# mafintosh/dat-replication-protocol

Hardware: AMD Instinct MI355X
Metric: decoded Change frames/sec + wire GB/s (whole node) at 1/2/4/8 MI355X (higher is better)
Workload: dtype u8

## Files before the change

### dat-replication-protocol_amd/csrc/drp_decode_spec.hip

```cpp
#include "drp_spec.h"

#include <algorithm>
#include <cstdio>
#include <cstdlib>
#include <vector>

namespace drp {
namespace spec {

#ifndef DRP_K1_WAVES
#define DRP_K1_WAVES 8
#endif
#ifndef DRP_EMIT_WAVES
#define DRP_EMIT_WAVES 5
#endif
#ifndef DRP_KSTRONG
#define DRP_KSTRONG 4
#endif
constexpr int KSTRONG = DRP_KSTRONG;
struct Img {
  const uint8_t *lds;
  const uint8_t *g;
  uint64_t A, se;
  bool local = true;
// ... 579 lines not shown
    const uint64_t L1 = H1 ? ((1ull << (63 - __builtin_clzll(H1))) - 1) : 0ull;
    const uint64_t L0 = H1 ? ~0ull : (H0 ? ((1ull << (63 - __builtin_clzll(H0))) - 1) : 0ull);
    S0 = H0 & ~(F0 & L0);
    S1 = H1 & ~(F1 & L1);
    if (far && any_above(H0, H1, tid)) {
      g = NONE;
      R = NONE;
      n = 0;
    }
  }
  uint64_t E = g;
  bool rs = false;
  PHASE(1);
  link<false>(m, s1, g, NONE, E, R, n, xr, xf, P.overflow, &rs);
  uint32_t need = (E == NONE && defer && !any_above(S0, S1, tid)) ? 1u : 0u;
  uint32_t js = (is_pos(E) && E < s1) ? tid + 1 : 0u;
  block_max2_u32(need, js, xf2);
  bool moved = false;
  for (uint32_t it = 0; need && it < 3; it++) {
    moved = true;
    if (E == NONE && defer && !any_above(S0, S1, tid)) {
      while (defer) {
        const uint32_t o = (uint32_t)__builtin_ctzll(defer);
        defer &= defer - 1;
        uint64_t r;
        uint32_t k;
        bool f;
        if (strong<false>(m, lb + o, s1, r, k, f, P.kstrong_hbm) == S_OK) {
          g = lb + o;
          E = g;
          R = r;
          n = k;
          break;
        }
      }
    }
    link<false>(m, s1, g, NONE, E, R, n, xr, xf, P.overflow, &rs);
    need = (E == NONE && defer && !any_above(S0, S1, tid)) ? 1u : 0u;
    js = (is_pos(E) && E < s1) ? tid + 1 : 0u;
    block_max2_u32(need, js, xf2);
  }
  PHASE(2);
  {
    bool after;
    if (!moved) {
      after = any_from(S0, S1, js);
    } else {
      after = block_max_u32(g != NONE && tid + 1 > js ? 1u : 0u, xf2) != 0;
    }
    if (js && after) {
      const uint64_t Ea = E, Ra = R;
      const uint32_t na = n;
      const bool rsa = rs;
      const bool mine = tid + 1 > js;
      E = NONE;
      R = NONE;
      n = 0;
      link<false>(m, s1, mine ? g : NONE, NONE, E, R, n, xr, xf, P.overflow, &rs);
      const uint32_t nb = block_sum_u32(mine ? (n & 0xFFFFu) : 0u, xf2);
      if (nb < 2 || !mine) {
        E = Ea;
        R = Ra;
        n = na;
        rs = rsa;
      }
    }
  }
  PHASE(3);
  {
    const bool carrier = is_pos(E) && E >= lb && E < s1 && E < G.se;
    const uint64_t ix = t * NT + tid;
    P.ent[ix] = carrier ? (uint8_t)((E - lb) | (rs ? 0x40u : 0u)) : (uint8_t)0xFF;
    P.ent_n[ix] = carrier ? (uint8_t)(n & 0xFFFFu) : (uint8_t)0;
    P.ent_c[ix] = carrier ? (uint8_t)(n >> 16) : (uint8_t)0;
  }
  if (tid == NT - 1) P.claim[t] = (R == NONE || ((R & MARK_TERM) && (R & M_ERR))) ? C_ID : R;
  }
}

#ifndef DRP_FCAP
#define DRP_FCAP 512
#endif
constexpr uint32_t FCAP = DRP_FCAP;
constexpr uint16_t NX_TAILB = 0xFFFB, NX_TAILC = 0xFFFC;
constexpr uint32_t RX_NONE = 0xFFFFFFFFu;
constexpr uint32_t RX_DEAD = 0xFFFFFFFEu;
constexpr uint32_t RX_FAR = 0x80000000u;
constexpr uint32_t RX_TERM = 0x40000000u;
static_assert(IMG < 0x4000, "node offsets are 14-bit");
__device__ __forceinline__ bool rx_node(uint32_t x) { return x < RX_TERM; }
__device__ __forceinline__ uint32_t rx_off(uint32_t x) { return x >> 16; }

__device__ __forceinline__ uint32_t le2_bytes(uint32_t x) { return ~(((x | 0x80808080u) - 0x03030303u) | x) & 0x80808080u; }
__device__ __forceinline__ uint32_t gather_msb(uint32_t a, uint32_t b, uint32_t c, uint32_t d) {
  const uint32_t lo = __builtin_amdgcn_udot4(a, 0x08040201u, __builtin_amdgcn_udot4(b, 0x80402010u, 0u, false), false);
  const uint32_t hi = __builtin_amdgcn_udot4(c, 0x08040201u, __builtin_amdgcn_udot4(d, 0x80402010u, 0u, false), false);
  return (lo >> 7) | (hi << 1);
}
__device__ __forceinline__ uint32_t masks16(const uint4 v) {
  constexpr uint32_t H = 0x80808080u;
  const uint32_t m = gather_msb(v.x & H, v.y & H, v.z & H, v.w & H);
  const uint32_t s = gather_msb(le2_bytes(v.x), le2_bytes(v.y), le2_bytes(v.z), le2_bytes(v.w));
  return m | (s << 16);
}


__device__ __forceinline__ bool change_fills(const uint32_t *w32, uint32_t po, uint32_t pl, uint32_t lim,
                                             uint32_t off = 0, uint32_t found = 0) {
#pragma unroll 1
  for (uint32_t f = 0; f < 8u && off < pl; f++) {
    const uint32_t q = po + off;
    if (q + 12u > lim) return false;
    const uint32_t d = q >> 2, sh = (q & 3u) * 8u;
    const uint32_t a0 = w32[d], a1 = w32[d + 1], a2 = w32[d + 2];
    const uint32_t w = __builtin_amdgcn_alignbit(a1, a0, sh), wn = __builtin_amdgcn_alignbit(a2, a1, sh);
    const uint32_t b0 = w & 0xFFu, tag = b0 >> 3;
    const bool num = tag - 3u <= 2u;
    if (b0 >= 0x80u || tag - 1u > 5u || (b0 & 7u) != (num ? 0u : 2u)) return false;
    const uint32_t x = __builtin_amdgcn_alignbit(wn, w, 8);
    const uint32_t tm = ~x & 0x80808080u;
    uint32_t k2;
    uint64_t v = (x & 0x7Fu) | ((x >> 1) & 0x3F80u) | ((x >> 2) & 0x1FC000u) | ((x >> 3) & 0xFE00000u);
    if (tm) {
      k2 = ((uint32_t)__builtin_ctz(tm) >> 3) + 1u;
      v &= (1u << (7u * k2)) - 1u;
    } else {
      const uint32_t b5 = (wn >> 8) & 0xFFu;
      if (b5 & 0x80u) return false;
      k2 = 5u;
      v |= (uint64_t)b5 << 28;
    }
    if (k2 + 1u > pl - off) return false;
    if (num) {
      found |= 1u << (tag - 2u);
      off += 1u + k2;
    } else {
      const uint32_t o2 = off + 1u + k2;
      if (v > (uint64_t)(pl - o2)) return false;
      if (tag == 2u) found |= 1u;
      off = o2 + (uint32_t)v;
    }
  }
  return off == pl && found == 15u;
}

__device__ __forceinline__ uint32_t change_fills_win(const uint32_t *w32, uint32_t po, uint32_t pl, uint32_t lim,
                                                     uint32_t off, uint32_t found) {
  const uint32_t q = po + off;
  if (q + 36u > lim) return 2u;
  const uint32_t d = q >> 2, sh = (q & 3u) * 8u;
  uint32_t a[9];
#pragma unroll
  for (int i = 0; i < 9; i++) a[i] = w32[d + i];
  uint64_t x[4];
#pragma unroll
  for (int i = 0; i < 4; i++)
    x[i] = (uint64_t)__builtin_amdgcn_alignbit(a[2 * i + 1], a[2 * i], sh) |
           ((uint64_t)__builtin_amdgcn_alignbit(a[2 * i + 2], a[2 * i + 1], sh) << 32);
  uint32_t used = 0;
#pragma unroll
  for (int f = 0; f < 4; f++) {
    const uint32_t b0 = (uint32_t)x[0] & 0xFFu, tag = b0 >> 3;
    const uint64_t y = x[0] >> 8;
    const uint64_t tm = ~y & 0x8080808080ull;
    if (b0 >= 0x80u || !tm) return 0u;
    const uint32_t k2 = ((uint32_t)__builtin_ctzll(tm) >> 3) + 1u;
    const uint64_t v = ((y & 0x7Full) | ((y >> 1) & 0x3F80ull) | ((y >> 2) & 0x1FC000ull) | ((y >> 3) & 0xFE00000ull) |
                        ((y >> 4) & 0x7F0000000ull)) & ((1ull << (7u * k2)) - 1ull);
    if (tag - 3u <= 2u && (b0 & 7u) == 0u) {
      found |= 1u << (tag - 2u);
      const uint32_t s = 1u + k2;
      used += s;
      if (off + used > pl) return 0u;
      const uint32_t b = 8u * s;
      x[0] = (x[0] >> b) | (x[1] << (64u - b));
      x[1] = (x[1] >> b) | (x[2] << (64u - b));
      x[2] = (x[2] >> b) | (x[3] << (64u - b));
      x[3] >>= b;
      continue;
    }
    if (b0 == 0x32u) {
      return (found == 15u && (uint64_t)off + used + 1u + k2 + v == (uint64_t)pl) ? 1u : 0u;
    }
    if (b0 == 0x0Au || b0 == 0x12u) return 2u;
    return 0u;
  }
  return 2u;
}

__device__ __forceinline__ uint32_t fwalk(const uint32_t *lnd, uint32_t x, uint32_t s1r, uint32_t &n) {
  n = 0;
  uint32_t i = x & 0xFFFFu;
#pragma unroll 1
  for (;;) {
    const uint32_t nd = lnd[i], id = nd >> 30, c = nd & 0xFFFFu, q = (nd >> 16) & 0x3FFFu;
    if (id == 3) return RX_DEAD;
    if (c == NX_TAILC) return RX_TERM | i;
    n += 1u + ((id == 1) << 16) - (id == 0);
    if (c == NX_TAILB) return RX_TERM | i;
    if (c == NX_FAR || c == NX_NEAR) return RX_FAR | i;
    if (q >= s1r) return c == NX_DEAD ? RX_DEAD : (c | (q << 16));
    if (c == NX_DEAD) return RX_DEAD;
    i = c;
  }
}

__device__ __forceinline__ bool flink(const uint32_t *lnd, uint32_t s1r, uint32_t g, uint32_t &E, uint32_t &R,
                                      uint32_t &n, bool &rs, uint32_t *wl, uint32_t *fl, uint32_t *overflow,
                                      unsigned long long *stats = nullptr, uint32_t cap = ~0u) {
  const uint32_t tid = threadIdx.x, lane = tid & 63u, wid = tid >> 6;
  const uint64_t below = (1ull << lane) - 1ull;
#pragma unroll 1
  for (uint32_t round = 0;; round++) {
    const bool carrier = rx_node(E) && rx_off(E) < s1r;
    const uint64_t cm = __ballot(carrier);
    const uint64_t bm = cm & below;
    const uint32_t j = bm ? 63u - (uint32_t)__builtin_clzll(bm) : 0u;
    const uint32_t xj = (uint32_t)__builtin_amdgcn_ds_bpermute((int)(j << 2), (int)R);
    if constexpr (NT == 2 * WAVE) {
      if (lane == 0) wl[wid] = cm ? (uint32_t)__builtin_amdgcn_readlane((int)R, 63 - __builtin_clzll(cm)) : RX_NONE;
      bsync();
    }
    const uint32_t prev = (NT == 2 * WAVE && wid == 1) ? wl[0] : RX_NONE;
    const uint32_t ex = bm ? xj : prev;
    const bool r = ex >= RX_DEAD;
    const uint32_t En = r ? g : ex;
    const bool ch = En != E;
    const bool relevant = ch && (carrier || (rx_node(En) && rx_off(En) < s1r));
    const uint64_t any = __ballot(relevant);
    bool more = any != 0;
    if constexpr (NT == 2 * WAVE) {
      if (lane == 0) fl[wid] = any != 0;
      bsync();
      more = (fl[0] | fl[1]) != 0;
    }
    rs = r;
    if (more && round + 1 >= cap) return true;
    if (!more) {
      if (stats && tid == 0) {
        atomicAdd(&stats[56], (unsigned long long)(round + 1));
        atomicMax(&stats[57], (unsigned long long)(round + 1));
        if (round + 1 > 8) atomicAdd(&stats[58], 1ull);
      }
      if (ch) {
        E = En;
        R = En;
        n = 0;
      }
      break;
    }
    if (round > NT + 2) {
      if (tid == 0) atomicOr(overflow, F_WAIT);
      break;
    }
    if (ch) {
      E = En;
      if (rx_node(E) && rx_off(E) < s1r) R = fwalk(lnd, E, s1r, n);
      else {
        R = E;
        n = 0;
      }
    }
  }
  return false;
}



constexpr uint32_t HV = HALO / SEGB;
struct FastLds {
  union {
    struct {
      uint64_t lmw[NT + HV];
      uint64_t dmw[NT];
      uint16_t loff[NT + HV];
      uint32_t hmx[HALO / 16 + 1];
      uint16_t lpos[FCAP];
      uint32_t lnd[FCAP > NT + 1 ? FCAP : NT + 1];
      uint8_t lal[FCAP];
      uint32_t lsucc[FCAP];
    };
    __attribute__((aligned(16))) uint8_t img[IMG + 32];
  };
  uint32_t fls[NT];
  uint32_t xw[8];
  uint32_t xf[2 * NT / WAVE], wl[NT / WAVE], fl[NT / WAVE];
  uint64_t xm[4];
#ifdef DRP_K1_PAD
  uint8_t pad[DRP_K1_PAD];
#endif
};
static_assert(sizeof(FastLds) <= SPEC_BUF, "spec_claims runs the edge form in its image buffer");


#ifndef DRP_FL_CAP
#define DRP_FL_CAP 6
#endif
constexpr uint32_t JT_C_ID = 2u << 30, JT_TERM = 1u << 30, JT_NONE = 0xFFFFu;
template <uint32_t NTT>
__device__ __forceinline__ uint32_t fast_claims_jump(const DecodeParams &P, uint64_t t, uint64_t A, FastLds &S, uint32_t g,
                                                  uint32_t ttotal, uint32_t total, uint32_t &eb_o, uint32_t &en_o,
                                                  uint32_t &ecn_o, uint64_t &cl_o) {
  const uint32_t tid = threadIdx.x, lane = tid & 63u, wid = tid >> 6;
  constexpr uint32_t KPT = FCAP / NTT;
  uint16_t *nx = reinterpret_cast<uint16_t *>(S.lmw);
  uint32_t *gl = reinterpret_cast<uint32_t *>(S.dmw);
  uint32_t *lnd = S.lnd;
  if (P.stats && tid == 0) atomicAdd(&P.stats[60], 1ull);
  const uint64_t gm = __ballot(g != RX_NONE);
  if (lane == 0) S.xm[wid] = gm;
  gl[tid] = g;
  bsync();
  const uint64_t G0 = S.xm[0], G1 = NTT == 2 * WAVE ? S.xm[1] : 0ull;
  uint32_t yn[KPT], yt[KPT];
#pragma unroll
  for (uint32_t j = 0; j < KPT; j++) {
    const uint32_t i = tid + j * NTT;
    yn[j] = JT_NONE;
    yt[j] = JT_C_ID;
    if (i < ttotal) {
      const uint32_t o = S.lpos[i], th = o / SEGB;
      uint32_t cnt;
      const uint32_t x = fwalk(lnd, i, (th + 1u) * SEGB, cnt);
      if (rx_node(x)) {
        const uint32_t k = x & 0xFFFFu;
        if (S.lpos[k] >= TILE) yt[j] = S.lpos[k];
        else yn[j] = k;
      } else if (x == RX_DEAD) {
        const uint64_t a0 = th + 1u < 64u ? G0 & (~0ull << (th + 1u)) : 0ull;
        const uint64_t a1 = th + 1u < 64u ? G1 : (th + 1u < 128u ? G1 & (~0ull << (th + 1u - 64u)) : 0ull);
        const uint32_t k = a0 ? (uint32_t)__builtin_ctzll(a0) : (a1 ? 64u + (uint32_t)__builtin_ctzll(a1) : NTT);
        if (k < NTT) yn[j] = gl[k] & 0xFFFFu;
      } else if (x & RX_FAR) {
        yt[j] = S.lsucc[x & 0xFFFFu];
      } else if (x & RX_TERM) {
        yt[j] = JT_TERM | S.lpos[x & 0xFFFFu];
      }
    } else if (i < total) {
      yt[j] = S.lpos[i];
    }
  }
  bsync();
#pragma unroll
  for (uint32_t j = 0; j < KPT; j++) {
    const uint32_t i = tid + j * NTT;
    if (i < total) {
      nx[i] = (uint16_t)yn[j];
      lnd[i] = yt[j];
    }
  }
  bsync();
#pragma unroll 1
  for (uint32_t round = 0; round < 10u; round++) {
    uint32_t chm = 0;
#pragma unroll
    for (uint32_t j = 0; j < KPT; j++) {
      const uint32_t i = tid + j * NTT;
      if (i < total && nx[i] != JT_NONE) {
        const uint32_t a = nx[i], b = nx[a];
        yn[j] = b;
        yt[j] = b == JT_NONE ? lnd[a] : 0u;
        chm |= 1u << j;
      }
    }
    const uint64_t any = __ballot(chm != 0);
    if (lane == 0) S.fl[wid] = any != 0;
    bsync();
    uint32_t more = 0;
#pragma unroll
    for (uint32_t w = 0; w < NTT / WAVE; w++) more |= S.fl[w];
#pragma unroll
    for (uint32_t j = 0; j < KPT; j++)
      if ((chm >> j) & 1u) {
        const uint32_t i = tid + j * NTT;
        nx[i] = (uint16_t)yn[j];
        if (yn[j] == JT_NONE) lnd[i] = yt[j];
      }
    bsync();
    if (!more) break;
  }
  const uint64_t ix = t * NTT + tid;
  eb_o = 0xFFu;
  en_o = 0;
  ecn_o = 0;
  P.ent[ix] = 0xFF;
  P.ent_n[ix] = 0;
  P.ent_c[ix] = 0;
  cl_o = 0;
  if (tid == NTT - 1) {
    uint64_t cl = C_ID;
    if (G0 | G1) {
      const uint32_t k = G0 ? (uint32_t)__builtin_ctzll(G0) : 64u + (uint32_t)__builtin_ctzll(G1);
      const uint32_t s0 = gl[k] & 0xFFFFu;
      const uint32_t code = nx[s0] == JT_NONE ? lnd[s0] : JT_C_ID;
      if (code == JT_C_ID) cl = C_ID;
      else if (code & JT_TERM) cl = MARK_TERM | (A + (code & ~JT_TERM));
      else cl = A + code;
    }
    P.claim[t] = cl;
    cl_o = cl;
  }
  return FC_OK;
}

#ifndef DRP_CREC_STAGE
#define DRP_CREC_STAGE 2
#endif
constexpr uint32_t CR_CAP = NT, CR_WORDS = 6, CR_TILE_WORDS = CR_CAP * CR_WORDS;
static_assert(CR_CAP == NT, "one frame per thread in the record decode");

__device__ __forceinline__ bool crec_general(const uint32_t *w32, uint32_t qa, uint32_t ke, uint32_t pl,
                                             uint32_t &num0, uint32_t &num1, uint32_t &num2, uint32_t &vo, bool &hv) {
  const uint32_t d = qa >> 2, sh = (qa & 3u) * 8u;
  uint32_t a[8];
#pragma unroll
  for (int i = 0; i < 8; i++) a[i] = w32[d + i];
  uint64_t x[4];
#pragma unroll
  for (int i = 0; i < 3; i++)
    x[i] = (uint64_t)__builtin_amdgcn_alignbit(a[2 * i + 1], a[2 * i], sh) |
           ((uint64_t)__builtin_amdgcn_alignbit(a[2 * i + 2], a[2 * i + 1], sh) << 32);
  x[3] = __builtin_amdgcn_alignbit(a[7], a[6], sh);
  uint32_t used = 0, nums[3];
#pragma unroll
  for (int f = 0; f < 3; f++) {
    const uint32_t b0 = (uint32_t)x[0] & 0xFFu;
    const uint64_t y = x[0] >> 8;
    const uint64_t tm = ~y & 0x8080808080ull;
    if (b0 != 0x18u + 8u * (uint32_t)f || !tm) return false;
    const uint32_t k2 = ((uint32_t)__builtin_ctzll(tm) >> 3) + 1u;
    const uint64_t v = ((y & 0x7Full) | ((y >> 1) & 0x3F80ull) | ((y >> 2) & 0x1FC000ull) | ((y >> 3) & 0xFE00000ull) |
                        ((y >> 4) & 0x7F0000000ull)) & ((1ull << (7u * k2)) - 1ull);
    if (v >> 32) return false;
    nums[f] = (uint32_t)v;
    const uint32_t s = 1u + k2, b = 8u * s;
    used += s;
    x[0] = (x[0] >> b) | (x[1] << (64u - b));
    x[1] = (x[1] >> b) | (x[2] << (64u - b));
    x[2] = (x[2] >> b) | (x[3] << (64u - b));
    x[3] >>= b;
  }
  num0 = nums[0];
  num1 = nums[1];
  num2 = nums[2];
  if (ke + used > pl) return false;
  hv = ke + used != pl;
  vo = 0;
  if (!hv) return true;
  const uint32_t b0 = (uint32_t)x[0] & 0xFFu;
  const uint64_t y = x[0] >> 8;
  const uint64_t tm = ~y & 0x80808080ull;
  if (b0 != 0x32u || !tm) return false;
  const uint32_t k2 = ((uint32_t)__builtin_ctzll(tm) >> 3) + 1u;
  const uint64_t v = ((y & 0x7Full) | ((y >> 1) & 0x3F80ull) | ((y >> 2) & 0x1FC000ull) | ((y >> 3) & 0xFE00000ull)) &
                     ((1ull << (7u * k2)) - 1ull);
  vo = ke + used + 1u + k2;
  return vo <= pl && v == (uint64_t)(pl - vo) && vo < 0x10000u;
}

__device__ __forceinline__ bool crec_frame(const uint32_t *w32, uint32_t o, uint32_t se_rel, uint32_t id, bool tailb,
                                           uint32_t (&w)[CR_WORDS]) {
  const uint32_t d = o >> 2, sh = (o & 3u) * 8u;
  const uint32_t a0 = w32[d], a1 = w32[d + 1], a2 = w32[d + 2];
  const uint32_t h = __builtin_amdgcn_alignbit(a1, a0, sh), hn = __builtin_amdgcn_alignbit(a2, a1, sh);
  const uint32_t k = ((uint32_t)__builtin_ctz((~h & 0x808080u) | 0x80000000u) >> 3) + 1u;
  const uint32_t L = ((h & 0x7Fu) | ((h >> 1) & 0x3F80u) | ((h >> 2) & 0x1FC000u)) & ((1u << (7u * k)) - 1u);
  const uint32_t po = o + k + 1u, pl = L - 1u;
  w[0] = po | (id << 14) | ((tailb ? 1u : 0u) << 16);
  w[1] = pl;
  w[2] = w[3] = w[4] = w[5] = 0;
  if (id != 1u) return true;
  const uint64_t x = (((uint64_t)hn << 32) | h) >> (8u * (k + 1u));
  const uint32_t b1 = (uint32_t)(x >> 8) & 0xFFu, b2 = (uint32_t)(x >> 16) & 0xFFu;
  const uint32_t kb = b1 < 0x80u ? 1u : (b2 < 0x80u ? 2u : 0u);
  const uint32_t klen = kb == 1u ? b1 : (b1 & 0x7Fu) | (b2 << 7);
  const uint32_t ke = 1u + kb + klen;
  uint32_t n0 = 0, n1 = 0, n2 = 0, vo = 0;
  bool hv = false, ok = ((uint32_t)x & 0xFFu) == 0x12u && kb && ke + 6u <= pl;
  const uint32_t qa = po + ke;
  ok = ok && qa + 36u <= se_rel;
  if (ok) {
    const uint32_t e = qa >> 2, s2 = (qa & 3u) * 8u;
    const uint32_t c0 = w32[e], c1 = w32[e + 1], c2 = w32[e + 2], c3 = w32[e + 3];
    const uint64_t y = (uint64_t)__builtin_amdgcn_alignbit(c1, c0, s2) | ((uint64_t)__builtin_amdgcn_alignbit(c2, c1, s2) << 32);
    const uint32_t y8 = __builtin_amdgcn_alignbit(c3, c2, s2) & 0xFFu;
    const bool one = (y & 0xFFull) == 0x18u && ((y >> 16) & 0xFFull) == 0x20u && ((y >> 32) & 0xFFull) == 0x28u &&
                     (y & 0x0000800080008000ull) == 0;
    if (one) {
      n0 = (uint32_t)(y >> 8) & 0xFFu;
      n1 = (uint32_t)(y >> 24) & 0xFFu;
      n2 = (uint32_t)(y >> 40) & 0xFFu;
      if (ke + 6u != pl) {
        const uint32_t d0 = (uint32_t)(y >> 56), vh = d0 < 0x80u ? 2u : (y8 < 0x80u ? 3u : 0u);
        const uint32_t vl = vh == 2u ? d0 : (d0 & 0x7Fu) | (y8 << 7);
        vo = ke + 6u + vh;
        hv = true;
        ok = ((uint32_t)(y >> 48) & 0xFFu) == 0x32u && vh && vo <= pl && vl == pl - vo && vo < 0x10000u;
      }
    } else {
      ok = crec_general(w32, qa, ke, pl, n0, n1, n2, vo, hv);
    }
  }
  w[0] |= ((hv ? 1u : 0u) << 17) | (kb << 18);
  w[2] = klen | (vo << 16);
  w[3] = n0;
  w[4] = n1;
  w[5] = n2;
  return ok;
}

__device__ __forceinline__ void fast_records(const DecodeParams &P, uint64_t t, FastLds &S, uint32_t E, uint32_t nf,
                                             uint32_t s1r, uint32_t se_rel, const uint4 (&v)[SEGB / 16],
                                             const uint4 &hv) {
  const uint32_t tid = threadIdx.x, lane = tid & 63u, wid = tid >> 6;
  const uint32_t ip = wave_scan_dpp(nf);
  if (lane == 63) S.xw[4 + wid] = ip;
  bsync();
  const uint32_t tot = NT == 2 * WAVE ? S.xw[4] + S.xw[5] : S.xw[4];
  if (tot > CR_CAP) return;
  uint32_t bad = 0;
  if (nf) {
    uint32_t slot = ip - nf + (wid ? S.xw[4] : 0u), cnt = 0, i = E & 0xFFFFu;
#pragma unroll 1
    for (uint32_t g = 0; g < 64u; g++) {
      const uint32_t nd = S.lnd[i], id = nd >> 30, c = nd & 0xFFFFu, q = (nd >> 16) & 0x3FFFu;
      if (id == 3u || c == NX_TAILC) break;
      if (id != 0u) {
        if (cnt < nf) S.fls[slot + cnt] = (uint32_t)S.lpos[i] | (id << 14) | ((c == NX_TAILB ? 1u : 0u) << 16);
        cnt++;
      }
      if (c >= NX_TAILB || q >= s1r) break;
      i = c;
    }
    bad = cnt != nf;
  }
  bsync();
  if (DRP_CREC_STAGE == 0) return;
  uint4 *im = reinterpret_cast<uint4 *>(S.img);
#pragma unroll
  for (uint32_t k = 0; k < SEGB / 16; k++) im[tid * (SEGB / 16) + k] = v[k];
  if (tid < HALO / 16) im[TILE / 16 + tid] = hv;
  if (tid < 2) im[IMG / 16 + tid] = make_uint4(0, 0, 0, 0);
  bsync();
  if (tid < tot && !bad) {
    const uint32_t f = S.fls[tid];
    uint32_t w[CR_WORDS];
    bad = !crec_frame(reinterpret_cast<const uint32_t *>(S.img), f & 0x3FFFu, min(se_rel, IMG), (f >> 14) & 3u,
                      (f >> 16) & 1u, w);
    uint32_t *rr = P.rec + t * CR_TILE_WORDS + tid;
    if (DRP_CREC_STAGE == 1) {
      if ((w[0] ^ w[2] ^ w[3] ^ w[4] ^ w[5]) == 0x7FFFFFFFu && !bad) rr[0] = w[1];
      bad = true;
    }
    if (!bad) {
      rr[0] = w[0];
      rr[CR_CAP] = w[1];
      if ((w[0] >> 14 & 3u) == 1u) {
#pragma unroll
        for (uint32_t k = 2; k < CR_WORDS; k++) rr[k * CR_CAP] = w[k];
      }
    }
  }
  const uint64_t bm = __ballot(bad);
  if (lane == 0) S.xw[6 + wid] = bm != 0;
  bsync();
  if (tid == 0) P.tile_rec[t] = (NT == 2 * WAVE ? S.xw[6] | S.xw[7] : S.xw[6]) ? REC_NONE : 0u;
}

__device__ __forceinline__ uint64_t range_bits(uint32_t base, uint32_t lo, uint32_t hi) {
  const uint32_t a = lo > base ? min(lo - base, 64u) : 0u, z = hi > base ? min(hi - base, 64u) : 0u;
  const uint64_t za = z >= 64u ? ~0ull : ((1ull << z) - 1ull), aa = a >= 64u ? ~0ull : ((1ull << a) - 1ull);
  return za & ~aa;
}

template <bool CF, bool EDGE, bool REC>
__device__ __forceinline__ uint32_t fast_claims(const DecodeParams &P, const TileGeo &G, uint64_t t, FastLds &S,
                                                uint32_t &eb_o, uint32_t &en_o, uint32_t &ecn_o, uint64_t &cl_o) {
  uint8_t *buf = nullptr;
  uint64_t *lmw = S.lmw, *dmw = S.dmw, *xm = S.xm;
  uint16_t *loff = S.loff, *lpos = S.lpos;
  uint32_t *hmx = S.hmx, *lnd = S.lnd, *xw = S.xw, *xf = S.xf, *wl = S.wl, *fl = S.fl;
  uint8_t *lal = S.lal;
  const uint32_t tid = threadIdx.x, lane = tid & 63u, wid = tid >> 6;
  uint4 v[SEGB / 16], hv;
  if (EDGE) {
    load_image(P, G, v, hv);
  } else {
    const uint4 *q = reinterpret_cast<const uint4 *>(P.bytes + G.A + (uint64_t)tid * SEGB);
#pragma unroll
    for (int k = 0; k < (int)(SEGB / 16); k++) v[k] = q[k];
    hv = tid < HALO / 16 ? *reinterpret_cast<const uint4 *>(P.bytes + G.A + TILE + tid * 16) : make_uint4(0, 0, 0, 0);
  }
  uint32_t mk[4];
#pragma unroll
  for (int k = 0; k < 4; k++) mk[k] = masks16(v[k]);
  uint32_t *mx = lnd;
  mx[tid] = mk[0];
  if (tid < HALO / 16) {
    const uint32_t hmk = masks16(hv);
    hmx[tid] = hmk;
    if (tid == 0) mx[NT] = hmk;
  }
  if (tid == HALO / 16) hmx[HALO / 16] = 0xFFFFu;
  bsync();
  const uint32_t nx = mx[tid + 1];
  const uint64_t M0 = (uint64_t)(mk[0] & 0xFFFFu) | ((uint64_t)(mk[1] & 0xFFFFu) << 16) |
                      ((uint64_t)(mk[2] & 0xFFFFu) << 32) | ((uint64_t)(mk[3] & 0xFFFFu) << 48);
  const uint64_t S0 = (uint64_t)(mk[0] >> 16) | ((uint64_t)(mk[1] >> 16) << 16) | ((uint64_t)(mk[2] >> 16) << 32) |
                      ((uint64_t)(mk[3] >> 16) << 48);
  const uint64_t M1 = nx & 0xFFFFu, S1 = nx >> 16;
  const uint64_t X0 = ~M0 & ((S0 >> 1) | (S1 << 63));
  const uint64_t X1 = ~M1 & (S1 >> 1);
  const uint64_t Xs1 = (X0 >> 1) | (X1 << 63), Xs2 = (X0 >> 2) | (X1 << 62), Ms1 = (M0 >> 1) | (M1 << 63);
  uint64_t live = X0 | (M0 & (Xs1 | (Ms1 & Xs2)));
  uint32_t lo_rel = 0, hi_rel = IMG, fo_rel = IMG;
  if (EDGE) {
    lo_rel = G.e0 > G.A ? (uint32_t)umin64(G.e0 - G.A, IMG) : 0u;
    hi_rel = (uint32_t)umin64(G.se - G.A, IMG);
    fo_rel = hi_rel < IMG ? max(lo_rel, hi_rel >= 3u ? hi_rel - 3u : 0u) : IMG;
    live = (live & range_bits(tid * SEGB, lo_rel, hi_rel)) | range_bits(tid * SEGB, fo_rel, hi_rel);
  }
  uint64_t hlive = 0;
  if (tid < HV) {
    uint32_t hk[5];
#pragma unroll
    for (int k = 0; k < 5; k++) hk[k] = hmx[tid * 4 + k];
    const uint64_t hM0 = (uint64_t)(hk[0] & 0xFFFFu) | ((uint64_t)(hk[1] & 0xFFFFu) << 16) |
                         ((uint64_t)(hk[2] & 0xFFFFu) << 32) | ((uint64_t)(hk[3] & 0xFFFFu) << 48);
    const uint64_t hS0 = (uint64_t)(hk[0] >> 16) | ((uint64_t)(hk[1] >> 16) << 16) | ((uint64_t)(hk[2] >> 16) << 32) |
                         ((uint64_t)(hk[3] >> 16) << 48);
    const uint64_t hM1 = hk[4] & 0xFFFFu, hS1 = hk[4] >> 16;
    const uint64_t hX0 = ~hM0 & ((hS0 >> 1) | (hS1 << 63)), hX1 = ~hM1 & (hS1 >> 1);
    const uint64_t hXs1 = (hX0 >> 1) | (hX1 << 63), hXs2 = (hX0 >> 2) | (hX1 << 62), hMs1 = (hM0 >> 1) | (hM1 << 63);
    hlive = hX0 | (hM0 & (hXs1 | (hMs1 & hXs2)));
    if (EDGE)
      hlive = (hlive & range_bits(TILE + tid * SEGB, lo_rel, hi_rel)) | range_bits(TILE + tid * SEGB, fo_rel, hi_rel);
    if (tid == HV - 1) hlive &= (1ull << (SEGB - 16)) - 1ull;
  }
  const uint32_t cnt = (uint32_t)__builtin_popcountll(live);
  const uint32_t cpre = wave_scan_dpp(cnt);
  const uint32_t hcnt = (uint32_t)__builtin_popcountll(hlive);
  uint32_t hpre = 0;
  if (wid == 0) hpre = wave_scan_dpp(hcnt);
  if (lane == 63) xw[wid] = cpre;
  if (tid == 63) xw[2] = hpre;
  lmw[tid] = live;
  if (tid < HV) lmw[NT + tid] = hlive;
  bsync();
  const uint32_t off = cpre - cnt + (wid ? xw[0] : 0u);
  const uint32_t ttotal = NT == 2 * WAVE ? xw[0] + xw[1] : xw[0];
  const uint32_t total = ttotal + xw[2];
  if (total > FCAP) {
    if (!EDGE) push_work(P, t);
    return FC_DENSE;
  }
  loff[tid] = (uint16_t)off;
  {
    uint64_t bits = live;
    uint32_t i = off;
    while (bits) {
      lpos[i++] = (uint16_t)(tid * SEGB + (uint32_t)__builtin_ctzll(bits));
      bits &= bits - 1;
    }
  }
  if (tid < HV) {
    uint64_t bits = hlive;
    uint32_t i = ttotal + hpre - hcnt;
    loff[NT + tid] = (uint16_t)i;
    while (bits) {
      lpos[i++] = (uint16_t)(TILE + tid * SEGB + (uint32_t)__builtin_ctzll(bits));
      bits &= bits - 1;
    }
  }
  bsync();
  const uint32_t se_rel = (uint32_t)umin64(G.se - G.A, 0x7FFFFFFFull);
  constexpr uint32_t KPT = FCAP / NT;
  uint32_t ncode[KPT], npos[KPT];
  uint32_t na[KPT];
  uint32_t chained = 0;
  uint32_t cfw[KPT];
  uint32_t cff[KPT];
  const uint32_t *w32 = reinterpret_cast<const uint32_t *>(P.bytes + G.A);
#pragma unroll
  for (uint32_t j = 0; j < KPT; j++) {
    const uint32_t i = tid + j * NT;
    ncode[j] = NX_DEAD;
    na[j] = 0;
    npos[j] = 0;
    cfw[j] = 0;
    cff[j] = 0;
    if (i < total) {
      const uint32_t o = lpos[i];
      uint32_t w, wn, k, L, id, succ;
      bool valid, tail, exact = false;
      if (EDGE && o + 16u > se_rel) {
        const Hdr h = hdr_global(P.bytes, G.A + o, G.se);
        exact = true;
        tail = h.kind == H_TAIL_HDR || h.kind == H_TAIL_CHANGE || h.kind == H_TAIL_BLOB;
        valid = h.kind == H_VALID || tail;
        id = h.kind == H_TAIL_HDR ? 1u : h.id;
        k = h.vlen;
        L = (uint32_t)umin64(h.L, 0xFFFFFFFFull);
        succ = h.kind == H_VALID ? (uint32_t)(h.succ - G.A) : o + 1u;
        w = wn = 0;
      } else {
        const uint32_t d = o >> 2, sh = (o & 3u) * 8u;
        const uint32_t a0 = w32[d], a1 = w32[d + 1], a2 = w32[d + 2];
        w = __builtin_amdgcn_alignbit(a1, a0, sh);
        wn = __builtin_amdgcn_alignbit(a2, a1, sh);
        const uint32_t tm = ~w & 0x808080u;
        k = ((uint32_t)__builtin_ctz(tm | 0x80000000u) >> 3) + 1u;
        const uint32_t L3 = (w & 0x7Fu) | ((w >> 1) & 0x3F80u) | ((w >> 2) & 0x1FC000u);
        L = L3 & ((1u << (7u * k)) - 1u);
        id = (w >> (8u * k)) & 0xFFu;
        succ = o + k + (id ? L : 1u);
        const uint32_t avail = se_rel - o;
        valid = id <= 2u && (id == 0u || L != 0u);
        tail = valid && id != 0u && L > avail - k;
      }
      uint32_t c = NX_DEAD, a = 0;
      if (valid && !tail && !exact && id == 1u && k >= 2u && succ <= IMG) {
        const uint32_t pb = k == 3u ? (wn & 0xFFu) : (w >> (8u * (k + 1u))) & 0xFFu;
        constexpr uint64_t TAGS = (1ull << 0x0a) | (1ull << 0x12) | (1ull << 0x18) | (1ull << 0x20) | (1ull << 0x28) |
                                  (1ull << 0x32);
        valid = pb < 64u && ((TAGS >> pb) & 1ull);
      }
      if (!valid) {
        c = NX_DEAD;
      } else if (tail) {
        c = id == 2u ? NX_TAILB : NX_TAILC;
      } else if (succ >= se_rel) {
        c = NX_NEAR;
        a = 1;
        S.lsucc[i] = succ;
      } else if (succ >= IMG - 16) {
        c = NX_FAR;
        a = 2;
        S.lsucc[i] = succ;
        if (CF && id == 1u && (o < TILE || L > HALO) && L - 1u < (1u << 18)) {
          const uint32_t x = k + 1u < 4u ? __builtin_amdgcn_alignbit(wn, w, 8u * (k + 1u)) : wn;
          const uint32_t tg = x & 0xFFu, lt = ~(x >> 8) & 0x808080u;
          if ((tg == 0x0Au || tg == 0x12u) && lt) {
            const uint32_t nb = ((uint32_t)__builtin_ctz(lt) >> 3) + 1u, y = x >> 8;
            const uint32_t v = ((y & 0x7Fu) | ((y >> 1) & 0x3F80u) | ((y >> 2) & 0x1FC000u)) & ((1u << (7u * nb)) - 1u);
            const uint32_t f1 = 1u + nb + v;
            if (f1 < L - 1u) cfw[j] = (o + k + 1u) | ((L - 1u) << 14), cff[j] = f1 | ((tg == 0x12u ? 1u : 0u) << 20);
          }
        }
      } else {
        const uint32_t th = succ / SEGB, b = succ % SEGB;
        const uint64_t lw = lmw[th];
        if ((lw >> b) & 1ull) {
          c = loff[th] + (uint32_t)__builtin_popcountll(lw & ((1ull << b) - 1ull));
// ... 11 lines not shown
  if (CF && wave_sum_dpp(chained) < 16u) {
#pragma unroll
    for (uint32_t j = 0; j < KPT; j++) {
      uint32_t cr = 0;
      if (cfw[j]) {
        const uint32_t lim = min(se_rel, IMG + 512u), po = cfw[j] & 0x3FFFu,
                       pl = cfw[j] >> 14;
        cr = change_fills_win(w32, po, pl, lim, cff[j] & 0xFFFFFu, cff[j] >> 20);
        if (cr == 2u) cr = change_fills(w32, po, pl, lim, cff[j] & 0xFFFFFu, cff[j] >> 20) ? 1u : 0u;
      }
      if (cr == 1u) {
        na[j] = 1;
        lal[tid + j * NT] = 1;
      }
    }
  }
  bsync();
  lmw[tid] = 0;
  dmw[tid] = 0;
#pragma unroll 1
  for (int r = 1; r < KSTRONG; r++) {
#pragma unroll
    for (uint32_t j = 0; j < KPT; j++) {
      if (na[j] == 1u && ncode[j] < NX_NEAR) {
        const uint32_t b = lal[ncode[j]];
        if (b != 1u) {
          na[j] = b;
          lal[tid + j * NT] = (uint8_t)b;
        }
      }
    }
    bsync();
  }
#pragma unroll
  for (uint32_t j = 0; j < KPT; j++) {
    if (na[j] && npos[j] < TILE) {
      const uint32_t o = npos[j];
      atomicOr((unsigned long long *)(na[j] == 1u ? &lmw[o / SEGB] : &dmw[o / SEGB]), 1ull << (o % SEGB));
    }
  }
  bsync();
  const uint64_t sm = lmw[tid];
  const uint32_t lb = tid * SEGB, s1r = lb + SEGB;
  uint32_t g = RX_NONE;
  uint64_t defer = dmw[tid];
  bool far = false;
  if (sm) {
    const uint32_t b = (uint32_t)__builtin_ctzll(sm);
    defer &= (1ull << b) - 1ull;
    const uint32_t gi = off + (uint32_t)__builtin_popcountll(live & ((1ull << b) - 1ull));
    g = gi | ((lb + b) << 16);
    const uint32_t gc = lnd[gi] & 0xFFFFu;
    far = gc == NX_FAR || gc == NX_NEAR;
  }
  uint32_t n = 0, R = RX_NONE;
  if (g != RX_NONE) R = fwalk(lnd, g, s1r, n);
  uint64_t S0m, S1m;
  {
    const uint64_t hm = __ballot(g != RX_NONE), fm = __ballot(g != RX_NONE && far);
    uint64_t H0 = hm, H1 = 0, F0 = fm, F1 = 0;
    if constexpr (NT == 2 * WAVE) {
      if (lane == 0) {
        xm[wid] = hm;
        xm[2 + wid] = fm;
      }
      bsync();
      H0 = xm[0];
      H1 = xm[1];
      F0 = xm[2];
      F1 = xm[3];
    }
    const uint64_t L1 = H1 ? ((1ull << (63 - __builtin_clzll(H1))) - 1) : 0ull;
    const uint64_t L0 = H1 ? ~0ull : (H0 ? ((1ull << (63 - __builtin_clzll(H0))) - 1) : 0ull);
    S0m = H0 & ~(F0 & L0);
    S1m = H1 & ~(F1 & L1);
    if (far && any_above(H0, H1, tid)) {
      g = RX_NONE;
      R = RX_NONE;
      n = 0;
    }
  }
  uint32_t E = g;
  bool rs = false;
  if (flink(lnd, s1r, g, E, R, n, rs, wl, fl, P.overflow, P.stats, DRP_FL_CAP)) {
    if (tid == 0) {
      uint32_t c = __hip_atomic_load(&P.counter[12], __ATOMIC_RELAXED, __HIP_MEMORY_SCOPE_AGENT);
      if (c < P.jump_min) c = atomicAdd(&P.counter[12], 1u);
      xw[6] = c;
    }
    bsync();
    if (xw[6] >= P.jump_min) return fast_claims_jump<NT>(P, t, G.A, S, g, ttotal, total, eb_o, en_o, ecn_o, cl_o);
    flink(lnd, s1r, g, E, R, n, rs, wl, fl, P.overflow, P.stats);
  }
  const Img m{buf, P.bytes, G.A, G.se, false};
  uint32_t need, js;
  block_any_last(E == RX_NONE && defer && !any_above(S0m, S1m, tid), rx_node(E) && rx_off(E) < s1r, need, js, xf);
  bool moved = false;
  if (P.stats && tid == 0 && need) atomicAdd(&P.stats[59], 1ull);
#pragma unroll 1
  for (uint32_t it = 0; need && it < 3; it++) {
    moved = true;
    if (E == RX_NONE && defer && !any_above(S0m, S1m, tid)) {
      while (defer) {
        const uint32_t o = (uint32_t)__builtin_ctzll(defer);
        defer &= defer - 1;
        uint64_t r;
        uint32_t k;
        bool f;
        if (strong<false>(m, G.A + lb + o, G.A + s1r, r, k, f, P.kstrong_hbm) == S_OK) {
          g = (off + (uint32_t)__builtin_popcountll(live & ((1ull << o) - 1ull))) | ((lb + o) << 16);
          E = g;
          R = fwalk(lnd, g, s1r, n);
          break;
        }
      }
    }
    flink(lnd, s1r, g, E, R, n, rs, wl, fl, P.overflow);
    block_any_last(E == RX_NONE && defer && !any_above(S0m, S1m, tid), rx_node(E) && rx_off(E) < s1r, need, js,
                   xf);
  }
  {
    bool after;
    if (!moved) after = any_from(S0m, S1m, js);
    else after = block_max_u32(g != RX_NONE && tid + 1 > js ? 1u : 0u, xf) != 0;
    if (js && after) {
      const uint32_t Ea = E, Ra = R, na0 = n;
      const bool rsa = rs;
      const bool mine = tid + 1 > js;
      E = RX_NONE;
      R = RX_NONE;
      n = 0;
      flink(lnd, s1r, mine ? g : RX_NONE, E, R, n, rs, wl, fl, P.overflow);
      const uint32_t nb = block_sum_u32(mine ? (n & 0xFFFFu) : 0u, xf);
      if (nb < 2 || !mine) {
        E = Ea;
        R = Ra;
        n = na0;
        rs = rsa;
      }
    }
  }
  {
    const bool carrier = rx_node(E) && rx_off(E) < s1r;
    const uint64_t ix = t * NT + tid;
    eb_o = carrier ? (((rx_off(E) - lb) & 63u) | (rs ? 0x40u : 0u)) : 0xFFu;
    en_o = carrier ? (n & 0xFFFFu) : 0u;
    ecn_o = carrier ? (n >> 16) : 0u;
    P.ent[ix] = (uint8_t)eb_o;
    P.ent_n[ix] = (uint8_t)en_o;
    P.ent_c[ix] = (uint8_t)ecn_o;
  }
  cl_o = 0;
  if (tid == NT - 1) {
    uint64_t cl = C_ID;
    if (R < RX_DEAD && !rx_node(R)) {
      const uint64_t p = G.A + lpos[R & 0xFFFFu];
      if (R & RX_FAR) {
        cl = G.A + S.lsucc[R & 0xFFFFu];
      } else {
        cl = MARK_TERM | p;
      }
    } else if (rx_node(R)) {
      cl = G.A + rx_off(R);
    }
    P.claim[t] = cl;
    cl_o = cl;
  }
  if (!EDGE && REC) fast_records(P, t, S, E, en_o, s1r, se_rel, v, hv);
  return FC_OK;
}

#ifndef DRP_K1_REC_WAVES
#define DRP_K1_REC_WAVES 7
#endif
template <bool CF, bool REC>
__global__ __launch_bounds__(NT, REC ? DRP_K1_REC_WAVES : DRP_K1_WAVES) void claims_fast(DecodeParams P) {
  __shared__ FastLds S;
  const uint64_t ntiles = P.tile_prefix[P.nstreams];
  const uint64_t t = blockIdx.x;
  if (REC && t == 0 && threadIdx.x == 0) P.counter[13] = 1u;
  const TileGeo G = tile_geo(P, t);
  if (t >= ntiles) return;
  if (G.A < G.so || G.A + IMG > G.se) {
    push_work(P, t);
    return;
  }
  uint32_t eb, en, ecn;
  uint64_t cl;
  (void)fast_claims<CF, false, REC>(P, G, t, S, eb, en, ecn, cl);
}

#ifndef DRP_CASCADE_HARD
#define DRP_CASCADE_HARD 1
#endif
constexpr uint32_t VL_HARD = 1u << 31;
#ifndef DRP_CASCADE_DIV
#define DRP_CASCADE_DIV 8
#endif
constexpr uint32_t VL_BLK = 256, VL_G = NT / 16;
#ifndef DRP_SP_FRAMES
#define DRP_SP_FRAMES 8
#endif
constexpr uint32_t SP_FRAMES = DRP_SP_FRAMES;
__device__ __forceinline__ uint32_t bytes_from(uint32_t s, uint32_t d) {
  return s <= 4u * d ? 0xFFFFFFFFu : (s >= 4u * d + 4u ? 0u : 0xFFFFFFFFu << (8u * (s - 4u * d)));
}
__device__ __forceinline__ uint32_t restart_bytes(uint32_t x) {
  const uint32_t y = (x & 0xC0C0C0C0u) ^ 0x40404040u;
  return msb4(~(((y & 0x7F7F7F7Fu) + 0x7F7F7F7Fu) | y) & 0x80808080u);
}
__global__ __launch_bounds__(VL_BLK) void verify_lite(DecodeParams P) {
  const uint32_t tid = threadIdx.x, r = tid & (VL_G - 1u), gb = (tid & 63u) & ~(VL_G - 1u);
  const uint64_t t = ((uint64_t)blockIdx.x * VL_BLK + tid) / VL_G;
  const uint64_t ntiles = P.tile_prefix[P.nstreams];
  if (t >= ntiles) return;
  const TileGeo G = tile_geo(P, t);
  const uint64_t ix = t * NT + 16u * r;
  const uint4 e4 = *reinterpret_cast<const uint4 *>(P.ent + ix);
  const uint4 n4 = *reinterpret_cast<const uint4 *>(P.ent_n + ix);
  const uint4 c4 = *reinterpret_cast<const uint4 *>(P.ent_c + ix);
  const uint64_t claim = P.claim[t];
  uint64_t et = G.e0;
  bool found = t == G.tf;
  for (uint32_t step = 0; !found && step < 4u; step++) {
    const int64_t j = (int64_t)t - 1 - (int64_t)(VL_G * step + r);
    const bool virt = j < (int64_t)G.tf;
    const uint64_t c = virt ? G.e0 : P.claim[j];
    const uint32_t gm = (uint32_t)(__ballot(virt || c != C_ID) >> gb) & ((1u << VL_G) - 1u);
    if (gm) {
      const uint32_t src = gb + (uint32_t)__builtin_ctz(gm);
      et = ((uint64_t)(uint32_t)__shfl((int)(uint32_t)(c >> 32), (int)src, WAVE) << 32) |
           (uint32_t)__shfl((int)(uint32_t)c, (int)src, WAVE);
      found = true;
    }
  }
  const bool bogus = is_pos(et) && et < G.A;
  const bool inside = is_pos(et) && !bogus && et < G.A + TILE;
  const uint32_t k = inside ? (uint32_t)((et - G.A) / SEGB) : NT;
  const uint32_t kr = k / 16u, ki = k % 16u;
  const uint32_t ew[4] = {e4.x, e4.y, e4.z, e4.w}, nw[4] = {n4.x, n4.y, n4.z, n4.w}, cw[4] = {c4.x, c4.y, c4.z, c4.w};
  uint32_t bad = 0, sf = 0, sc = 0, rsm = 0, multi = 0, sb = 0;
  const uint32_t s = r > kr ? 0u : (r == kr ? ki : 16u);
#pragma unroll
  for (uint32_t d = 0; d < 4; d++) {
    const uint32_t m = bytes_from(s, d);
    sf = __builtin_amdgcn_udot4(nw[d] & m, 0x01010101u, sf, false);
    sc = __builtin_amdgcn_udot4(cw[d] & m, 0x01010101u, sc, false);
    sb = __builtin_amdgcn_udot4(nw[d] & ~m, 0x01010101u, sb, false);
// ... 1785 lines not shown
```

### dat-replication-protocol_amd/csrc/drp_spec.h

```cpp
#pragma once
#include "drp_device.h"
#include "drp_kernels.h"

namespace drp {
namespace spec {

#ifndef DRP_SPEC_NT
#define DRP_SPEC_NT 128
#endif
constexpr int NT = DRP_SPEC_NT;
constexpr uint32_t SEGB = 64;
constexpr uint32_t TILE = NT * SEGB;
static_assert(NT == 64 || NT == 128, "one or two waves per tile");

__device__ __forceinline__ void bsync() {
  if constexpr (NT == 64) asm volatile("s_waitcnt lgkmcnt(0)" ::: "memory");
  else __syncthreads();
}
constexpr uint32_t HALO = 512;
constexpr uint32_t IMG = TILE + HALO;

constexpr uint64_t RDY = 1ull << 63;
constexpr uint64_t C_ID = 1ull << 62;
constexpr uint64_t M_ERR = 1ull << 60;
constexpr uint64_t NONE = ~0ull;
constexpr uint32_t REC_NONE = 0xFFFFFFFFu;

constexpr uint32_t F_MISS = 1u << 12;
constexpr uint32_t F_WAIT = 1u << 13;
constexpr uint32_t F_CASCADE = 1u << 14;

__device__ __forceinline__ Hdr parse_win(uint64_t w0, uint64_t w1, uint64_t p, uint64_t se) {
  Hdr h;
  h.succ = 0;
  h.id = 0;
  const uint64_t avail = se - p;
  const uint32_t b0 = (uint32_t)(w0 & 0xFF);
  if (b0 < 0x80u && avail >= 2) {
    const uint32_t id = (uint32_t)((w0 >> 8) & 0xFF);
    h.L = b0;
    h.vlen = 1;
    h.id = id;
    if (id >= 3) { h.kind = H_ERR_TYPE; return h; }
    if (id == 0) { h.kind = H_VALID; h.succ = p + 2; return h; }
    if (b0 == 0) { h.kind = H_ERR_LEN; return h; }
    if ((uint64_t)b0 > avail - 1) { h.kind = (id == 1) ? H_TAIL_CHANGE : H_TAIL_BLOB; return h; }
    h.kind = H_VALID;
    h.succ = p + 1 + b0;
    return h;
  }
  uint64_t L;
  const int k = win_varint(w0, w1, 0, avail, L);
  h.L = L;
  h.vlen = (uint32_t)(k > 0 ? k : 0);
  if (k == 0) { h.kind = H_TAIL_HDR; return h; }
  if (k < 0) { h.kind = (avail < 11) ? H_TAIL_HDR : H_ERR_VARINT; return h; }
  if ((uint64_t)k >= avail) { h.kind = H_TAIL_HDR; return h; }
  const uint32_t id = win_byte(w0, w1, (uint32_t)k);
  h.id = id;
  if (id >= 3) { h.kind = H_ERR_TYPE; return h; }
  if (id == 0) { h.kind = H_VALID; h.succ = p + (uint64_t)k + 1; return h; }
  if (L == 0) { h.kind = H_ERR_LEN; return h; }
  if (L > avail - (uint64_t)k) { h.kind = (id == 1) ? H_TAIL_CHANGE : H_TAIL_BLOB; return h; }
  h.kind = H_VALID;
  h.succ = p + (uint64_t)k + L;
  return h;
}

__device__ __forceinline__ uint64_t funnel(uint64_t lo, uint64_t hi, uint32_t sh) {
  return sh ? (lo >> sh) | (hi << (64 - sh)) : lo;
}
__device__ __forceinline__ uint4 ld16(const uint8_t *g, uint64_t p, uint64_t se) {
  if (p + 16 <= se) return *reinterpret_cast<const uint4 *>(g + p);
  uint32_t w[4] = {0, 0, 0, 0};
  for (uint32_t k = 0; k < 16; k++)
    if (p + k < se) w[k >> 2] |= (uint32_t)g[p + k] << (8 * (k & 3));
  return make_uint4(w[0], w[1], w[2], w[3]);
}


__device__ __forceinline__ bool is_pos(uint64_t v) { return v < (1ull << 60); }

template <class T>
__device__ __forceinline__ T ldc(const T *p) {
  return *reinterpret_cast<const __attribute__((address_space(4))) T *>(reinterpret_cast<uintptr_t>(p));
}

struct TileGeo {
  uint64_t s, tf, so, se, A, e0;
};
__device__ __forceinline__ TileGeo tile_geo(const DecodeParams &P, uint64_t t) {
  TileGeo G;
  G.s = P.tile_stream ? ldc(P.tile_stream + t) : 0;
  if (G.s >= P.nstreams) G.s = P.nstreams - 1;
  G.tf = ldc(P.tile_prefix + G.s);
  G.so = ldc(P.stream_off + G.s);
  G.se = ldc(P.stream_off + G.s + 1);
  G.A = (G.so & ~(uint64_t)(TILE - 1)) + (t - G.tf) * TILE;
  G.e0 = G.so + (P.entry ? ldc(P.entry + G.s) : 0ull);
  return G;
}

__device__ __forceinline__ void push_work(const DecodeParams &P, uint64_t t) {
  if (threadIdx.x == 0) P.work[atomicAdd(P.work_n, 1u)] = (uint32_t)t;
}

__device__ __forceinline__ Hdr hdr_global(const uint8_t *g, uint64_t p, uint64_t se) {
  uint64_t w0, w1;
  const uint64_t a = p & ~15ull;
  const uint4 u = ld16(g, a, se), v = ld16(g, a + 16, se);
  const uint64_t q0 = ((uint64_t)u.y << 32) | u.x, q1 = ((uint64_t)u.w << 32) | u.z;
  const uint64_t q2 = ((uint64_t)v.y << 32) | v.x, q3 = ((uint64_t)v.w << 32) | v.z;
  const uint32_t o = (uint32_t)(p & 15);
  if (o < 8) {
    w0 = funnel(q0, q1, 8 * o);
    w1 = funnel(q1, q2, 8 * o);
  } else {
    w0 = funnel(q1, q2, 8 * (o - 8));
    w1 = funnel(q2, q3, 8 * (o - 8));
  }
  return parse_win(w0, w1, p, se);
}


constexpr uint32_t HOP_FRAME = 512;
__device__ __forceinline__ bool walk_hops(const DecodeParams &P) { return P.walk_hop == 1u; }

}
}
```

Baseline: 19.12 billion.

## Reload kernel args from kernarg segment and split halo liveness into 16-bit lanes

Kernel parameter fields (ent, claim, rec, counter, jump_min, overflow, kstrong_hbm) are now read straight from the kernarg segment at the point of use, behind an opaque asm barrier. This keeps them from being held in scalar registers across the long kernel and is meant to reduce register pressure. The halo liveness computation now gives each thread a 16-bit chunk built from two mask words instead of a 64-bit segment built from five, which spreads the halo work across more threads and shortens each one's serial ctz loop. A compile-time option can move this halo work to the second wave. Costs are extra scalar loads for the arguments and more threads doing halo work.

```diff
diff --git a/dat-replication-protocol_amd/csrc/drp_decode_spec.hip b/dat-replication-protocol_amd/csrc/drp_decode_spec.hip
--- a/dat-replication-protocol_amd/csrc/drp_decode_spec.hip
+++ b/dat-replication-protocol_amd/csrc/drp_decode_spec.hip
@@ -685,6 +685,9 @@
 #define DRP_FCAP 512
 #endif
 constexpr uint32_t FCAP = DRP_FCAP;
+#ifndef DRP_HALO_WAVE
+#define DRP_HALO_WAVE 0
+#endif
 constexpr uint16_t NX_TAILB = 0xFFFB, NX_TAILC = 0xFFFC;
 constexpr uint32_t RX_NONE = 0xFFFFFFFFu;
 constexpr uint32_t RX_DEAD = 0xFFFFFFFEu;
@@ -705,6 +708,11 @@
   const uint32_t m = gather_msb(v.x & H, v.y & H, v.z & H, v.w & H);
   const uint32_t s = gather_msb(le2_bytes(v.x), le2_bytes(v.y), le2_bytes(v.z), le2_bytes(v.w));
   return m | (s << 16);
+}
+__host__ __device__ __forceinline__ uint32_t halo_live16(uint32_t w, uint32_t wn) {
+  const uint32_t m = (w & 0xFFFFu) | (wn << 16), s = (w >> 16) | (wn & 0xFFFF0000u);
+  const uint32_t X = ~m & (s >> 1);
+  return (X | (m & ((X >> 1) | ((m >> 1) & (X >> 2))))) & 0xFFFFu;
 }
 
 
@@ -809,7 +817,7 @@
 }
 
 __device__ __forceinline__ bool flink(const uint32_t *lnd, uint32_t s1r, uint32_t g, uint32_t &E, uint32_t &R,
-                                      uint32_t &n, bool &rs, uint32_t *wl, uint32_t *fl, uint32_t *overflow,
+                                      uint32_t &n, bool &rs, uint32_t *wl, uint32_t *fl,
                                       unsigned long long *stats = nullptr, uint32_t cap = ~0u) {
   const uint32_t tid = threadIdx.x, lane = tid & 63u, wid = tid >> 6;
   const uint64_t below = (1ull << lane) - 1ull;
@@ -853,7 +861,7 @@
       break;
     }
     if (round > NT + 2) {
-      if (tid == 0) atomicOr(overflow, F_WAIT);
+      if (tid == 0) atomicOr(DRP_KARG(overflow), F_WAIT);
       break;
     }
     if (ch) {
@@ -986,9 +994,9 @@
   eb_o = 0xFFu;
   en_o = 0;
   ecn_o = 0;
-  P.ent[ix] = 0xFF;
-  P.ent_n[ix] = 0;
-  P.ent_c[ix] = 0;
+  DRP_KARG(ent)[ix] = 0xFF;
+  DRP_KARG(ent_n)[ix] = 0;
+  DRP_KARG(ent_c)[ix] = 0;
   cl_o = 0;
   if (tid == NTT - 1) {
     uint64_t cl = C_ID;
@@ -1000,7 +1008,7 @@
       else if (code & JT_TERM) cl = MARK_TERM | (A + (code & ~JT_TERM));
       else cl = A + code;
     }
-    P.claim[t] = cl;
+    DRP_KARG(claim)[t] = cl;
     cl_o = cl;
   }
   return FC_OK;
@@ -1150,7 +1158,7 @@
     uint32_t w[CR_WORDS];
     bad = !crec_frame(reinterpret_cast<const uint32_t *>(S.img), f & 0x3FFFu, min(se_rel, IMG), (f >> 14) & 3u,
                       (f >> 16) & 1u, w);
-    uint32_t *rr = P.rec + t * CR_TILE_WORDS + tid;
+    uint32_t *rr = DRP_KARG(rec) + t * CR_TILE_WORDS + tid;
     if (DRP_CREC_STAGE == 1) {
       if ((w[0] ^ w[2] ^ w[3] ^ w[4] ^ w[5]) == 0x7FFFFFFFu && !bad) rr[0] = w[1];
       bad = true;
@@ -1167,7 +1175,7 @@
   const uint64_t bm = __ballot(bad);
   if (lane == 0) S.xw[6 + wid] = bm != 0;
   bsync();
-  if (tid == 0) P.tile_rec[t] = (NT == 2 * WAVE ? S.xw[6] | S.xw[7] : S.xw[6]) ? REC_NONE : 0u;
+  if (tid == 0) DRP_KARG(tile_rec)[t] = (NT == 2 * WAVE ? S.xw[6] | S.xw[7] : S.xw[6]) ? REC_NONE : 0u;
 }
 
 __device__ __forceinline__ uint64_t range_bits(uint32_t base, uint32_t lo, uint32_t hi) {
@@ -1223,32 +1231,24 @@
     fo_rel = hi_rel < IMG ? max(lo_rel, hi_rel >= 3u ? hi_rel - 3u : 0u) : IMG;
     live = (live & range_bits(tid * SEGB, lo_rel, hi_rel)) | range_bits(tid * SEGB, fo_rel, hi_rel);
   }
-  uint64_t hlive = 0;
-  if (tid < HV) {
-    uint32_t hk[5];
-#pragma unroll
-    for (int k = 0; k < 5; k++) hk[k] = hmx[tid * 4 + k];
-    const uint64_t hM0 = (uint64_t)(hk[0] & 0xFFFFu) | ((uint64_t)(hk[1] & 0xFFFFu) << 16) |
-                         ((uint64_t)(hk[2] & 0xFFFFu) << 32) | ((uint64_t)(hk[3] & 0xFFFFu) << 48);
-    const uint64_t hS0 = (uint64_t)(hk[0] >> 16) | ((uint64_t)(hk[1] >> 16) << 16) | ((uint64_t)(hk[2] >> 16) << 32) |
-                         ((uint64_t)(hk[3] >> 16) << 48);
-    const uint64_t hM1 = hk[4] & 0xFFFFu, hS1 = hk[4] >> 16;
-    const uint64_t hX0 = ~hM0 & ((hS0 >> 1) | (hS1 << 63)), hX1 = ~hM1 & (hS1 >> 1);
-    const uint64_t hXs1 = (hX0 >> 1) | (hX1 << 63), hXs2 = (hX0 >> 2) | (hX1 << 62), hMs1 = (hM0 >> 1) | (hM1 << 63);
-    hlive = hX0 | (hM0 & (hXs1 | (hMs1 & hXs2)));
+  constexpr uint32_t HB = HALO / 16, HW0 = (NT == 2 * WAVE && DRP_HALO_WAVE) ? WAVE : 0u;
+  const uint32_t hl = tid - HW0;
+  uint32_t hlive = 0;
+  if (hl < HB - 1u) {
+    hlive = halo_live16(hmx[hl], hmx[hl + 1]);
     if (EDGE)
-      hlive = (hlive & range_bits(TILE + tid * SEGB, lo_rel, hi_rel)) | range_bits(TILE + tid * SEGB, fo_rel, hi_rel);
-    if (tid == HV - 1) hlive &= (1ull << (SEGB - 16)) - 1ull;
+      hlive = (hlive & (uint32_t)range_bits(TILE + hl * 16u, lo_rel, hi_rel) & 0xFFFFu) |
+              ((uint32_t)range_bits(TILE + hl * 16u, fo_rel, hi_rel) & 0xFFFFu);
   }
   const uint32_t cnt = (uint32_t)__builtin_popcountll(live);
   const uint32_t cpre = wave_scan_dpp(cnt);
-  const uint32_t hcnt = (uint32_t)__builtin_popcountll(hlive);
+  const uint32_t hcnt = (uint32_t)__builtin_popcount(hlive);
   uint32_t hpre = 0;
-  if (wid == 0) hpre = wave_scan_dpp(hcnt);
+  if (wid == HW0 / WAVE) hpre = wave_scan_dpp(hcnt);
   if (lane == 63) xw[wid] = cpre;
-  if (tid == 63) xw[2] = hpre;
+  if (tid == HW0 + 63u) xw[2] = hpre;
   lmw[tid] = live;
-  if (tid < HV) lmw[NT + tid] = hlive;
+  if (hl < HB) reinterpret_cast<uint16_t *>(lmw + NT)[hl] = (uint16_t)hlive;
   bsync();
   const uint32_t off = cpre - cnt + (wid ? xw[0] : 0u);
   const uint32_t ttotal = NT == 2 * WAVE ? xw[0] + xw[1] : xw[0];
@@ -1266,12 +1266,12 @@
       bits &= bits - 1;
     }
   }
-  if (tid < HV) {
-    uint64_t bits = hlive;
+  if (hl < HB) {
+    uint32_t bits = hlive;
     uint32_t i = ttotal + hpre - hcnt;
-    loff[NT + tid] = (uint16_t)i;
+    if (!(hl & 3u)) loff[NT + hl / 4u] = (uint16_t)i;
     while (bits) {
-      lpos[i++] = (uint16_t)(TILE + tid * SEGB + (uint32_t)__builtin_ctzll(bits));
+      lpos[i++] = (uint16_t)(TILE + hl * 16u + (uint32_t)__builtin_ctz(bits));
       bits &= bits - 1;
     }
   }
@@ -1449,15 +1449,16 @@
   }
   uint32_t E = g;
   bool rs = false;
-  if (flink(lnd, s1r, g, E, R, n, rs, wl, fl, P.overflow, P.stats, DRP_FL_CAP)) {
+  if (flink(lnd, s1r, g, E, R, n, rs, wl, fl, P.stats, DRP_FL_CAP)) {
     if (tid == 0) {
-      uint32_t c = __hip_atomic_load(&P.counter[12], __ATOMIC_RELAXED, __HIP_MEMORY_SCOPE_AGENT);
-      if (c < P.jump_min) c = atomicAdd(&P.counter[12], 1u);
+      uint32_t *c12 = DRP_KARG(counter) + 12;
+      uint32_t c = __hip_atomic_load(c12, __ATOMIC_RELAXED, __HIP_MEMORY_SCOPE_AGENT);
+      if (c < DRP_KARG(jump_min)) c = atomicAdd(c12, 1u);
       xw[6] = c;
     }
     bsync();
-    if (xw[6] >= P.jump_min) return fast_claims_jump<NT>(P, t, G.A, S, g, ttotal, total, eb_o, en_o, ecn_o, cl_o);
-    flink(lnd, s1r, g, E, R, n, rs, wl, fl, P.overflow, P.stats);
+    if (xw[6] >= DRP_KARG(jump_min)) return fast_claims_jump<NT>(P, t, G.A, S, g, ttotal, total, eb_o, en_o, ecn_o, cl_o);
+    flink(lnd, s1r, g, E, R, n, rs, wl, fl, P.stats);
   }
   const Img m{buf, P.bytes, G.A, G.se, false};
   uint32_t need, js;
@@ -1474,7 +1475,7 @@
         uint64_t r;
         uint32_t k;
         bool f;
-        if (strong<false>(m, G.A + lb + o, G.A + s1r, r, k, f, P.kstrong_hbm) == S_OK) {
+        if (strong<false>(m, G.A + lb + o, G.A + s1r, r, k, f, DRP_KARG(kstrong_hbm)) == S_OK) {
           g = (off + (uint32_t)__builtin_popcountll(live & ((1ull << o) - 1ull))) | ((lb + o) << 16);
           E = g;
           R = fwalk(lnd, g, s1r, n);
@@ -1482,7 +1483,7 @@
         }
       }
     }
-    flink(lnd, s1r, g, E, R, n, rs, wl, fl, P.overflow);
+    flink(lnd, s1r, g, E, R, n, rs, wl, fl);
     block_any_last(E == RX_NONE && defer && !any_above(S0m, S1m, tid), rx_node(E) && rx_off(E) < s1r, need, js,
                    xf);
   }
@@ -1497,7 +1498,7 @@
       E = RX_NONE;
       R = RX_NONE;
       n = 0;
-      flink(lnd, s1r, mine ? g : RX_NONE, E, R, n, rs, wl, fl, P.overflow);
+      flink(lnd, s1r, mine ? g : RX_NONE, E, R, n, rs, wl, fl);
       const uint32_t nb = block_sum_u32(mine ? (n & 0xFFFFu) : 0u, xf);
       if (nb < 2 || !mine) {
         E = Ea;
@@ -1513,9 +1514,9 @@
     eb_o = carrier ? (((rx_off(E) - lb) & 63u) | (rs ? 0x40u : 0u)) : 0xFFu;
     en_o = carrier ? (n & 0xFFFFu) : 0u;
     ecn_o = carrier ? (n >> 16) : 0u;
-    P.ent[ix] = (uint8_t)eb_o;
-    P.ent_n[ix] = (uint8_t)en_o;
-    P.ent_c[ix] = (uint8_t)ecn_o;
+    DRP_KARG(ent)[ix] = (uint8_t)eb_o;
+    DRP_KARG(ent_n)[ix] = (uint8_t)en_o;
+    DRP_KARG(ent_c)[ix] = (uint8_t)ecn_o;
   }
   cl_o = 0;
   if (tid == NT - 1) {
@@ -1530,7 +1531,7 @@
     } else if (rx_node(R)) {
       cl = G.A + rx_off(R);
     }
-    P.claim[t] = cl;
+    DRP_KARG(claim)[t] = cl;
     cl_o = cl;
   }
   if (!EDGE && REC) fast_records(P, t, S, E, en_o, s1r, se_rel, v, hv);
diff --git a/dat-replication-protocol_amd/csrc/drp_spec.h b/dat-replication-protocol_amd/csrc/drp_spec.h
--- a/dat-replication-protocol_amd/csrc/drp_spec.h
+++ b/dat-replication-protocol_amd/csrc/drp_spec.h
@@ -86,6 +86,14 @@
   return *reinterpret_cast<const __attribute__((address_space(4))) T *>(reinterpret_cast<uintptr_t>(p));
 }
 
+template <class T>
+__device__ __forceinline__ T karg_at(uint32_t off) {
+  uintptr_t k = reinterpret_cast<uintptr_t>(__builtin_amdgcn_kernarg_segment_ptr());
+  asm volatile("" : "+s"(k));
+  return *reinterpret_cast<const __attribute__((address_space(4))) T *>(k + off);
+}
+#define DRP_KARG(field) karg_at<decltype(DecodeParams::field)>((uint32_t)offsetof(DecodeParams, field))
+
 struct TileGeo {
   uint64_t s, tf, so, se, A, e0;
 };
```

Result: faster. 19.34 billion, median of 6 (+1.1%).
